# NVIDIAGameWorks/RayTracingDenoiser

Measured on AMD Instinct MI355X. Metric: Mpixels/s REBLUR_DIFFUSE_SPECULAR @1440p, higher is better.
Workload: dtype f32; 1 GPU; REBLUR_DIFFUSE_SPECULAR 2560x1440, default settings, analytic scene + 1rpp noise, moving camera; parallelism=1 GPU, storage=reference pool formats (fp16 history, R10G10B10A2 normals)

## Files before the change

raytracingdenoiser_amd/csrc/hip/kernels_reblur_history.hip:

```cpp
#include "passes.h"
#include "reblur_device.h"

namespace nrdhip {

constexpr int TILE_X = 32;
constexpr int TILE_Y = 8;

static const char* CheckSupportedHistory(const ReblurCB& c) {
    if (c.gRectOrigin.x != 0 || c.gRectOrigin.y != 0)
        return "internal error: a pass was handed a non-zero rectOrigin";
    if (c.gOrthoMode != 0.0f)
        return "REBLUR: orthographic projection is not supported (SURVEY.md section 8c)";
    return nullptr;
}

static_assert(TILE_X == 32 && TILE_Y == 8, "planes.h LoadBlockTileBytes: a workgroup covers two 16x16 tiles of one tile row");

namespace hf {
constexpr int BORDER = 2;
constexpr int BUF_X = TILE_X + 2 * BORDER;
constexpr int BUF_Y = TILE_Y + 2 * BORDER;
constexpr int BUF_STRIDE = BUF_X + 1;
}

struct HfPlanes {
    Plane tiles, normalRoughness, data1, viewZ, inDiff, inSpec, inDiffFast, inSpecFast, outDiff, outSpec, outDiffFast, outSpecFast;
    Plane inDiffSh, inSpecSh, outDiffSh, outSpecSh;
    NormalRoughnessGuide decodedNR;
};

struct HfPixel {
    int px, py, tx, ty;
    float viewZ, roughness, materialID, frustumSize;
    float3 N, Nv, Xv;
    float2 pixelUv;
};

template <bool IS_SPEC, bool DIFF, bool SPEC, bool PERF, int KIND, bool SH>
NRD_D typename ReblurSignal<KIND>::type HistoryFixSignal(const ReblurCB& c, const HfPlanes& P, const HfPixel& s, typename ReblurSignal<KIND>::type sig, float frameNum, float strideBase,
    const Plane& gIn_Signal, const Plane& gIn_Fast, const Plane& gOut_Fast, const float* s_Luma, float4& sh, const Plane& gIn_Sh) {
    typedef ReblurSignal<KIND> Sig;
    typedef typename Sig::type S;
    const int rw = c.gRectSizeMinusOne.x, rh = c.gRectSizeMinusOne.y;
    const float smc = GetSpecMagicCurve(s.roughness);

    float stride = strideBase * (frameNum < c.gHistoryFixFrameNum ? 1.0f : 0.0f);
    if (IS_SPEC)
        stride *= Lerp(0.5f, 1.0f, smc);
    stride = floorf(stride);

    if (stride != 0.0f) {
        const int stridei = (int)(stride + 0.5f);
        const float nonLinearAccumSpeed = Rcp(1.0f + frameNum);
        const float r = IS_SPEC ? s.roughness : 1.0f;
        const float2 rectSizeInv = ToF2(c.gRectSizeInv);
        const float4 hitDistParams = ToF4(c.gHitDistParams);

        float normalWeightParam = GetNormalWeightParam(nonLinearAccumSpeed, c.gLobeAngleFraction, r);
        float2 geometryWeightParams = GetGeometryWeightParams(c.gPlaneDistSensitivity, s.frustumSize, s.Xv, s.Nv);
        float2 relaxedRoughnessWeightParams = GetRelaxedRoughnessWeightParams(s.roughness * s.roughness, Sqrt(c.gRoughnessFraction));

        float hitDistScale = GetHitDistanceNormalization(s.viewZ, hitDistParams, r);
        float hitDist = ExtractHitDist(sig) * hitDistScale;
        float hitDistFactor = GetHitDistFactor(hitDist, s.frustumSize);
        float2 hitDistanceWeightParams = GetHitDistanceWeightParams(hitDistFactor, nonLinearAccumSpeed, r);

        float sumw = 1.0f + frameNum;
        if (PERF)
            sumw = 1.0f + Rcp(1.0f + c.gMaxAccumulatedFrameNum) - nonLinearAccumSpeed;
        sig = sig * sumw;
        if (SH)
            sh = F4(sh.x * sumw, sh.y * sumw, sh.z * sumw, IS_SPEC ? sh.w : sh.w * sumw);

        for (int j = -2; j <= 2; j++) {
            for (int i = -2; i <= 2; i++) {
                if ((i == 0 && j == 0) || (abs(i) + abs(j) == 4))
                    continue;

                float2 uv = s.pixelUv + F2(float(i), float(j)) * stride * rectSizeInv;
                int sx = ClampI(s.px + i * stridei, 0, rw), sy = ClampI(s.py + j * stridei, 0, rh);

                float zs = UnpackViewZ(c, LoadR32F(P.viewZ, sx, sy));
                float materialIDs;
                float4 Ns = LoadDecodedNormalRoughness(P.decodedNR, sx, sy, materialIDs);

                float angle = AcosApprox(Dot(Xyz(Ns), s.N));
                float3 Xvs = ReconstructViewPosition(uv, ToF4(c.gFrustum), zs, NRD_ORTHO_MODE(c));

                float w = IsInScreenNearest(uv);
                w *= ComputeWeight(Dot(s.Nv, Xvs), geometryWeightParams.x, geometryWeightParams.y);
                w *= CompareMaterials(s.materialID, materialIDs, IS_SPEC ? c.gSpecMinMaterial : c.gDiffMinMaterial) ? 1.0f : 0.0f;
                w *= ComputeExponentialWeight(angle, normalWeightParam, 0.0f);
                if (IS_SPEC)
                    w *= ComputeExponentialWeight(Ns.w * Ns.w, relaxedRoughnessWeightParams.x, relaxedRoughnessWeightParams.y);

                if (!PERF) {
                    float2 d1 = LoadData1<DIFF, SPEC>(P.data1, sx, sy);
                    w *= 1.0f + (IS_SPEC ? d1.y : d1.x);
                }

                S smp = Sig::Load(gIn_Signal, sx, sy);
                smp = Select(w == 0.0f, Sig::Zero(), smp);

                float hs = ExtractHitDist(smp) * hitDistScale;
                float hsFactor = GetHitDistFactor(hs, s.frustumSize);
                w *= ComputeExponentialWeight(hsFactor, hitDistanceWeightParams.x, hitDistanceWeightParams.y);

                if (IS_SPEC) {
                    float d = Div(Abs(hitDist - hs), Max(hitDist, hs) + 0.001f);
                    float b = LinearStep(0.03f, 0.05f, s.roughness);
                    w *= SmoothStep(0.2f + b, 0.05f + b, d);
                }

                sumw += w;
                sig = Mad(smp, w, sig);
                if (SH) {
                    float4 t = LoadRGBA16F(gIn_Sh, sx, sy);
                    t = Select(w == 0.0f, F4(0.0f), t);
                    sh = F4(sh.x + t.x * w, sh.y + t.y * w, sh.z + t.z * w, IS_SPEC ? sh.w : sh.w + t.w * w);
                }
            }
        }

        sumw = PositiveRcp(sumw);
        sig = sig * sumw;
        if (SH)
            sh = F4(sh.x * sumw, sh.y * sumw, sh.z * sumw, IS_SPEC ? sh.w : sh.w * sumw);
    }

    float center = s_Luma[(s.ty + hf::BORDER) * hf::BUF_STRIDE + s.tx + hf::BORDER];
    float m1 = center, m2 = center * center;

    float f = Sat(Div(frameNum, c.gHistoryFixFrameNum + NRD_EPS));
    if (IS_SPEC)
        f = Lerp(1.0f, f, smc);
    center = Lerp(GetLuma(sig), center, f);
    Sig::StoreFast(gOut_Fast, s.px, s.py, center);

#pragma unroll
    for (int j = 0; j <= 4; j++) {
#pragma unroll
        for (int i = 0; i <= 4; i++) {
            if (i == 2 && j == 2)
                continue;
            float d = s_Luma[(s.ty + j) * hf::BUF_STRIDE + s.tx + i];
            m1 += d;
            m2 += d * d;
        }
    }

    float luma = GetLuma(sig);

    if (KIND == SIGNAL_RADIANCE && c.gAntiFirefly != 0.0f) {
        float am1 = 0.0f, am2 = 0.0f;
        const int R = PERF ? 3 : REBLUR_ANTI_FIREFLY_FILTER_RADIUS;
        for (int j = -R; j <= R; j++)
            for (int i = -R; i <= R; i++) {
                if (abs(i) <= 1 && abs(j) <= 1)
                    continue;
                float d = LoadR16F(gIn_Fast, ClampI(s.px + i, 0, rw), ClampI(s.py + j, 0, rh));
                am1 += d;
                am2 += d * d;
            }
        float invNorm = Rcp(float((R * 2 + 1) * (R * 2 + 1) - 3 * 3));
        am1 *= invNorm;
        am2 *= invNorm;
        float sigma = Sqrt(Abs(am2 - am1 * am1)) * REBLUR_ANTI_FIREFLY_SIGMA_SCALE;
        luma = Clamp(luma, am1 - sigma, am1 + sigma);
    }

    m1 = m1 * (1.0f / 25.0f);
    m2 = m2 * (1.0f / 25.0f);
    float sigma = Sqrt(Abs(m2 - m1 * m1)) * (KIND != SIGNAL_RADIANCE ? REBLUR_COLOR_CLAMPING_SIGMA_SCALE_OCCLUSION : REBLUR_COLOR_CLAMPING_SIGMA_SCALE);
    float lumaClamped = Clamp(luma, m1 - sigma, m1 + sigma);
    luma = Lerp(lumaClamped, luma, Rcp(1.0f + (c.gMaxFastAccumulatedFrameNum < c.gMaxAccumulatedFrameNum ? 1.0f : 0.0f) * frameNum * 2.0f));

    if (SH) {
        float k = GetLumaScale(Length(Xyz(sh)), luma);
        sh = F4(sh.x * k, sh.y * k, sh.z * k, sh.w);
    }
    return ChangeLuma(sig, luma);
}

#ifndef NRD_REBLUR_HF_ROTATE
#define NRD_REBLUR_HF_ROTATE 1
#endif
template <bool DIFF, bool SPEC, bool PERF, int KIND, bool SH>
__global__ __launch_bounds__(TILE_X* TILE_Y, SH ? 0 : NRD_WAVES_REBLUR_HF) void ReblurHistoryFixKernel(ReblurCB c, HfPlanes P, RowRange rr) {
    typedef ReblurSignal<KIND> Sig;
    typedef typename Sig::type S;
    __shared__ float s_DiffLuma[DIFF ? hf::BUF_Y * hf::BUF_STRIDE : 1];
    __shared__ float s_SpecLuma[SPEC ? hf::BUF_Y * hf::BUF_STRIDE : 1];

    const int tx = threadIdx.x % TILE_X, ty = threadIdx.x / TILE_X;
    const int blockY = BlockTileY(rr);
    const int tileX = NRD_REBLUR_HF_ROTATE ? BlockTileXRotated(rr, blockY) : BlockTileX(rr);
    const int px = tileX * TILE_X + tx, py = blockY * TILE_Y + ty;
    const int rw = c.gRectSizeMinusOne.x, rh = c.gRectSizeMinusOne.y;

    const uint32_t tileBytes = LoadBlockTileBytes(P.tiles, tileX, blockY);
    if (!TileBytesHaveGeometry<2>(tileBytes))
        return;
    const int qx = min(px, rw), qy = min(max(py, 0), rh);
    const bool preSky = TileByteIsSky(tileBytes, tx >> 4);
    const float preViewZ = LoadR32F(P.viewZ, qx, qy);
    float preMaterialID;
    const float4 preNormalAndRoughness = LoadDecodedNormalRoughness(P.decodedNR, qx, qy, preMaterialID);
    const float2 preData1 = LoadData1<DIFF, SPEC>(P.data1, qx, qy);
    S preDiff = Sig::Zero(), preSpec = Sig::Zero();
    if (DIFF)
        preDiff = Sig::Load(P.inDiff, qx, qy);
    if (SPEC)
        preSpec = Sig::Load(P.inSpec, qx, qy);
    {
        const int baseX = tileX * TILE_X - hf::BORDER, baseY = blockY * TILE_Y - hf::BORDER;
        for (int i = threadIdx.x; i < hf::BUF_X * hf::BUF_Y; i += TILE_X * TILE_Y) {
            int lx = i % hf::BUF_X, ly = i / hf::BUF_X;
            int gx = ClampI(baseX + lx, 0, rw), gy = ClampI(baseY + ly, 0, rh);
            if (DIFF)
                s_DiffLuma[ly * hf::BUF_STRIDE + lx] = Sig::LoadFast(P.inDiffFast, gx, gy);
            if (SPEC)
                s_SpecLuma[ly * hf::BUF_STRIDE + lx] = Sig::LoadFast(P.inSpecFast, gx, gy);
        }
    }
    __syncthreads();

    if (px > rw || py > rh || py < rr.rowBegin || py >= rr.rowEnd)
        return;
    if (preSky)
        return;
    HfPixel s;
    s.viewZ = UnpackViewZ(c, preViewZ);
    if (s.viewZ > c.gDenoisingRange)
        return;

    s.px = px, s.py = py, s.tx = tx, s.ty = ty;
    s.materialID = preMaterialID;
    float4 normalAndRoughness = preNormalAndRoughness;
    s.N = Xyz(normalAndRoughness);
    s.roughness = normalAndRoughness.w;
    s.frustumSize = GetFrustumSize(c.gMinRectDimMulUnproject, NRD_ORTHO_MODE(c), s.viewZ);
    s.pixelUv = F2(float(px) + 0.5f, float(py) + 0.5f) * ToF2(c.gRectSizeInv);
    s.Xv = ReconstructViewPosition(s.pixelUv, ToF4(c.gFrustum), s.viewZ, NRD_ORTHO_MODE(c));
    s.Nv = RotateVectorInverse(c.gViewToWorld, s.N);
    float2 frameNum = preData1;
    float2 stride = F2(Div(c.gHistoryFixBasePixelStride, 2.0f + frameNum.x), Div(c.gHistoryFixBasePixelStride, 2.0f + frameNum.y));

    if (DIFF) {
        float4 diffSh = F4(0.0f);
        if (SH)
            diffSh = LoadRGBA16F(P.inDiffSh, px, py);
        S diff = HistoryFixSignal<false, DIFF, SPEC, PERF, KIND, SH>(c, P, s, preDiff, frameNum.x, stride.x, P.inDiff, P.inDiffFast, P.outDiffFast, s_DiffLuma, diffSh, P.inDiffSh);
        Sig::Store(P.outDiff, px, py, diff);
        if (SH)
            StoreRGBA16F(P.outDiffSh, px, py, diffSh);
    }
    if (SPEC) {
        float4 specSh = F4(0.0f);
        if (SH)
            specSh = LoadRGBA16F(P.inSpecSh, px, py);
        S spec = HistoryFixSignal<true, DIFF, SPEC, PERF, KIND, SH>(c, P, s, preSpec, frameNum.y, stride.y, P.inSpec, P.inSpecFast, P.outSpecFast, s_SpecLuma, specSh, P.inSpecSh);
        Sig::Store(P.outSpec, px, py, spec);
        if (SH)
            StoreRGBA16F(P.outSpecSh, px, py, specSh);
    }
}

template <bool DIFF, bool SPEC, bool PERF, int KIND, bool SH>
static const char* LaunchHistoryFix(const PassArgs& a) {
    const ReblurCB& c = *(const ReblurCB*)a.constants;
    if (const char* err = CheckSupportedHistory(c))
        return err;
    HfPlanes P = {};
    uint32_t k = 0;
    P.tiles = a.planes[k++];
    P.normalRoughness = a.planes[k++];
    if (const char* err = MakeNormalRoughnessGuide(a, P.decodedNR))
        return err;
    P.data1 = a.planes[k++];
    P.viewZ = a.planes[k++];
    if (DIFF) P.inDiff = a.planes[k++];
    if (SPEC) P.inSpec = a.planes[k++];
    if (DIFF) P.inDiffFast = a.planes[k++];
    if (SPEC) P.inSpecFast = a.planes[k++];
    if (DIFF && SH) P.inDiffSh = a.planes[k++];
    if (SPEC && SH) P.inSpecSh = a.planes[k++];
    if (DIFF) P.outDiff = a.planes[k++];
    if (SPEC) P.outSpec = a.planes[k++];
    if (DIFF) P.outDiffFast = a.planes[k++];
    if (SPEC) P.outSpecFast = a.planes[k++];
    if (DIFF && SH) P.outDiffSh = a.planes[k++];
    if (SPEC && SH) P.outSpecSh = a.planes[k++];
    if (k != a.planesNum)
        return "REBLUR history fix: unexpected resource count";
    RowGrid g = GridForRows(c.gRectSizeMinusOne.x + 1, c.gRectSizeMinusOne.y + 1, TILE_X, TILE_Y, a.rowBegin, a.rowEnd);
    LaunchPass(a, (ReblurHistoryFixKernel<DIFF, SPEC, PERF, KIND, SH>), g.grid, dim3(TILE_X * TILE_Y), c, P, MakeRowRange(g));
    return nullptr;
}

namespace ts {
constexpr int BORDER = 1;
constexpr int BUF_X = TILE_X + 2 * BORDER;
constexpr int BUF_Y = TILE_Y + 2 * BORDER;
constexpr int BUF_STRIDE = BUF_X + 1;
}

struct TsPlanes {
    Plane tiles, normalRoughness, viewZ, data1, data2, inDiff, inSpec, historyDiffLuma, historySpecLuma, inSpecHitDistForTracking, mv, outInternalData, outDiff, outSpec, outDiffLuma,
        outSpecLuma;
    Plane inDiffSh, inSpecSh, outDiffSh, outSpecSh;
    NormalRoughnessGuide decodedNR;
    Plane baseColorMetalness;
};

template <bool PERF>
NRD_D void LumaStats(const ReblurCB& c, const float* s_Luma, int tx, int ty, float& luma, float& m1, float& sigma) {
    luma = s_Luma[(ty + ts::BORDER) * ts::BUF_STRIDE + tx + ts::BORDER];
    float M1 = luma, M2 = luma * luma, mn = NRD_INF, mx = -NRD_INF;
#pragma unroll
    for (int j = 0; j <= 2; j++) {
#pragma unroll
        for (int i = 0; i <= 2; i++) {
            if (i == 1 && j == 1)
                continue;
            float d = s_Luma[(ty + j) * ts::BUF_STRIDE + tx + i];
            M1 += d;
            M2 += d * d;
            mn = Min(mn, d);
            mx = Max(mx, d);
        }
    }
    M1 = M1 * (1.0f / 9.0f);
    M2 = M2 * (1.0f / 9.0f);
    m1 = M1;
    sigma = Sqrt(Abs(M2 - M1 * M1));
    if (!PERF && c.gMaxBlurRadius != 0.0f)
        luma = Clamp(luma, mn, mx);
}

template <bool DIFF, bool SPEC, bool PERF, bool SH, int KIND, bool MVMOD>
__global__ __launch_bounds__(TILE_X* TILE_Y, NRD_WAVES_REBLUR_TS) void ReblurTemporalStabilizationKernel(ReblurCB c, TsPlanes P, RowRange rr) {
    typedef ReblurSignal<KIND> Sig;
    typedef typename Sig::type S;
    __shared__ float s_DiffLuma[DIFF ? ts::BUF_Y * ts::BUF_STRIDE : 1];
    __shared__ float s_SpecLuma[SPEC ? ts::BUF_Y * ts::BUF_STRIDE : 1];

    const int tx = threadIdx.x % TILE_X, ty = threadIdx.x / TILE_X;
    const int blockY = BlockTileY(rr, NRD_ALT_TILE_ORDER != 0);
    const int px = BlockTileX(rr) * TILE_X + tx, py = blockY * TILE_Y + ty;
// ... 281 lines not shown
```

raytracingdenoiser_amd/csrc/hip/kernels_relax_spatial.hip:

```cpp
#include "relax_device.h"

namespace nrdhip {

namespace {

constexpr int TILE_X = RELAX_TILE_X;
constexpr int TILE_Y = RELAX_TILE_Y;

__device__ __constant__ const float g_Poisson8[8][3] = {
    {-0.4706069f, -0.4427112f, +0.6461146f}, {-0.9057375f, +0.3003471f, +0.9542373f}, {-0.3487388f, +0.4037880f, +0.5335386f}, {+0.1023042f, +0.6439373f, +0.6520134f},
    {+0.5699277f, +0.3513750f, +0.6695386f}, {+0.2939128f, -0.1131226f, +0.3149309f}, {+0.7836658f, -0.4208784f, +0.8895339f}, {+0.1564120f, -0.8198990f, +0.8346850f}};

__device__ __constant__ const float g_Poisson8Gaussian[8] = {0.7591725f, 0.5482766f, 0.8287159f, 0.7553454f, 0.743887f, 0.9366367f, 0.59319115f, 0.6313964f};

__global__ __launch_bounds__(256) void RelaxClassifyTilesKernel(Plane viewZ, Plane tiles, float denoisingRange, int tilesPerRow, int tileRows) {
    const int wave = threadIdx.x >> 6, lane = threadIdx.x & 63;
    const int tileIndex = blockIdx.x * 4 + wave;
    if (tileIndex >= tilesPerRow * tileRows)
        return;
    const int tx = tileIndex % tilesPerRow, ty = tileIndex / tilesPerRow;
    const int x = tx * 16 + (lane & 3) * 4, y = ty * 16 + (lane >> 2);

    bool allSky = true;
    if (y < viewZ.h && x + 3 < viewZ.w) {
// ... 397 lines not shown
            StoreRGBA16FHinted<NT>(P.spec.outSh, px, py, Clamp4(specularSH, -NRD_FP16_MAX, NRD_FP16_MAX));
    }
}

template <bool DIFF, bool SPEC, bool SH>
const char* LaunchPrePass(const PassArgs& a) {
    if (const char* e = CheckSupportedRelax(a))
        return e;
    PlaneCursor cur(a);
    PrePassPlanes P = {};
    P.tiles = cur.next();
    if (SPEC) P.spec.in = cur.next();
    if (DIFF) P.diff.in = cur.next();
    P.normalRoughness = cur.next();
    P.viewZ = cur.next();
    if (SH && SPEC) P.spec.inSh = cur.next();
    if (SH && DIFF) P.diff.inSh = cur.next();
    if (SPEC) P.spec.out = cur.next();
    if (DIFF) P.diff.out = cur.next();
    if (SH && SPEC) P.spec.outSh = cur.next();
    if (SH && DIFF) P.diff.outSh = cur.next();
    P.decodedNR = a.decodedNormalRoughness;
    P.worldPos = a.worldPosViewZ;
    if (!cur.complete() || !P.decodedNR.ptr)
        return "RELAX PrePass: unexpected resource count or missing decoded normal/roughness cache";
    RelaxCB c = LoadRelaxConstants(a);
    RowGrid g = GridForRows(c.shared.gRectSize.x, c.shared.gRectSize.y, TILE_X, TILE_Y, a.rowBegin, a.rowEnd);
    const char* forceGeneric = getenv("NRD_HIP_GENERIC_TAPS");
    const bool fullRect = c.shared.gResolutionScale.x == 1.0f && c.shared.gResolutionScale.y == 1.0f && c.shared.gRectSize.x == P.decodedNR.w &&
                          c.shared.gRectSize.y == P.decodedNR.h && P.viewZ.w == P.decodedNR.w && P.viewZ.h == P.decodedNR.h && !(forceGeneric && atoi(forceGeneric) != 0);
    if ((SPEC && c.shared.gSpecCheckerboard != 2u) || (DIFF && c.shared.gDiffCheckerboard != 2u))
        LaunchPass(a, (RelaxPrePassKernel<DIFF, SPEC, SH, true, false>), g.grid, dim3(256), P, c, MakeRowRange(g));
    else if (fullRect && !(c.shared.gSpecMinMaterial < 3.0f || c.shared.gDiffMinMaterial < 3.0f) && (uint32_t)P.decodedNR.w * (uint32_t)P.decodedNR.h > NRD_NT_STORE_PIXELS)
        LaunchPass(a, (RelaxPrePassKernel<DIFF, SPEC, SH, false, true, false, true>), g.grid, dim3(256), P, c, MakeRowRange(g));
    else if (fullRect && !(c.shared.gSpecMinMaterial < 3.0f || c.shared.gDiffMinMaterial < 3.0f))
        LaunchPass(a, (RelaxPrePassKernel<DIFF, SPEC, SH, false, true, false>), g.grid, dim3(256), P, c, MakeRowRange(g));
    else if (fullRect)
        LaunchPass(a, (RelaxPrePassKernel<DIFF, SPEC, SH, false, true>), g.grid, dim3(256), P, c, MakeRowRange(g));
    else
        LaunchPass(a, (RelaxPrePassKernel<DIFF, SPEC, SH, false, false>), g.grid, dim3(256), P, c, MakeRowRange(g));
    return nullptr;
}

struct HistoryFixPlanes {
    Plane tiles, historyLength, normalRoughness, viewZ;
    Plane decodedNR;
    SignalPlanes spec, diff;
};

#ifndef NRD_RELAX_HF_ROTATE
#define NRD_RELAX_HF_ROTATE 1
#endif
template <bool DIFF, bool SPEC, bool SH>
__global__ __launch_bounds__(256, NRD_WAVES_RELAX_HF) void RelaxHistoryFixKernel(HistoryFixPlanes P, RelaxCB c, RowRange rows) {
    const int blockY = BlockTileY(rows, false) ;
    const int tileX = NRD_RELAX_HF_ROTATE ? BlockTileXRotated(rows, blockY) : BlockTileX(rows);
    const uint32_t tileBytes = LoadBlockTileBytes(P.tiles, tileX, blockY);
    if (!TileBytesHaveGeometry<2>(tileBytes))
        return;
    const int px = tileX * TILE_X + (threadIdx.x & 31), py = blockY * TILE_Y + (threadIdx.x >> 5);
    const int rectW = c.shared.gRectSize.x, rectH = c.shared.gRectSize.y;
    if (px >= rectW || py >= rectH || py < rows.rowBegin || py >= rows.rowEnd)
        return;
    float centerViewZ = RelaxUnpackViewZ(c, LoadR32F(P.viewZ, px, py));
    float historyLength = 255.0f * LoadR8Unorm(P.historyLength, px, py);
    if (TileByteIsSky(tileBytes, (threadIdx.x & 31) >> 4))
        return;
    if (centerViewZ > c.shared.gDenoisingRange || (historyLength > c.shared.gHistoryFixFrameNum || c.shared.gHistoryFixFrameNum == 1.0f))
        return;

    float centerMaterialID;
    float4 centerNormalRoughness = LoadDecodedNormalRoughness(P.decodedNR, px, py, centerMaterialID);
    float3 centerNormal = Xyz(centerNormalRoughness);
    float centerRoughness = centerNormalRoughness.w;
    float3 centerWorldPos = GetCurrentWorldPosFromPixelPos(c, px, py, centerViewZ);
    float3 centerV = -Normalize(centerWorldPos);
    float depthThreshold = c.shared.gDepthThreshold * centerViewZ;

    float4 diffuseSum = DIFF ? LoadRGBA16F(P.diff.in, px, py) : F4(0.0f);
    float4 diffuseSumSH = (DIFF && SH) ? LoadRGBA16F(P.diff.inSh, px, py) : F4(0.0f);
    float diffuseWSum = 1.0f;
    float4 specularSum = SPEC ? LoadRGBA16F(P.spec.in, px, py) : F4(0.0f);
    float4 specularSumSH = (SPEC && SH) ? LoadRGBA16F(P.spec.inSh, px, py) : F4(0.0f);
    float roughnessModified = specularSumSH.w;
    float specularWSum = 1.0f;
    float2 specularNormalWeightParams = SPEC ? GetNormalWeightParams_ATrous(centerRoughness, 5.0f, 1.0f, 0.0f, c.shared.gLobeAngleFraction, c.shared.gSpecLobeAngleSlack) : F2(0.0f, 0.0f);
    const float normalPower = Max(c.shared.gHistoryFixEdgeStoppingNormalPower, 0.01f);

    float r = Div(c.shared.gHistoryFixBasePixelStride, 1.0f + historyLength);
    r = floorf(r + 0.5f);

    for (int j = -2; j <= 2; j++)
        for (int i = -2; i <= 2; i++) {
            int dx = (int)(float(i) * r), dy = (int)(float(j) * r);
            int sx = px + dx, sy = py + dy;
            bool isInside = sx >= 0 && sy >= 0 && sx < rectW && sy < rectH;
            if (i == 0 && j == 0)
                continue;

            float sampleMaterialID;
            float3 sampleNormal = Xyz(LoadDecodedNormalRoughnessOrZero(P.decodedNR, sx, sy, sampleMaterialID));
            float sampleViewZ = RelaxUnpackViewZ(c, LoadR32FOrZero(P.viewZ, sx, sy));
            float3 sampleWorldPos = GetCurrentWorldPosFromPixelPos(c, sx, sy, sampleViewZ);
            float geometryWeight = GetPlaneDistanceWeight_Atrous(centerWorldPos, centerNormal, sampleWorldPos, depthThreshold);

            if (DIFF) {
                float diffuseW = geometryWeight;
                diffuseW *= Pow(Max(0.01f, Dot(centerNormal, sampleNormal)), normalPower);
                diffuseW = isInside ? diffuseW : 0.0f;
                diffuseW *= Cmp(CompareMaterials(sampleMaterialID, centerMaterialID, c.shared.gDiffMinMaterial));
                if (diffuseW > 1e-4f) {
                    diffuseSum = diffuseSum + LoadRGBA16FOrZero(P.diff.in, sx, sy) * diffuseW;
                    if (SH)
                        diffuseSumSH = diffuseSumSH + LoadRGBA16FOrZero(P.diff.inSh, sx, sy) * diffuseW;
                    diffuseWSum += diffuseW;
                }
            }
            if (SPEC) {
                float3 sampleV = -Normalize(sampleWorldPos + c.shared.gRoughnessEdgeStoppingRelaxation * centerWorldPos);
                float specularW = geometryWeight;
                specularW *= GetSpecularNormalWeight_ATrous(specularNormalWeightParams, centerNormal, sampleNormal, centerV, sampleV);
                specularW = isInside ? specularW : 0.0f;
                specularW *= Cmp(CompareMaterials(sampleMaterialID, centerMaterialID, c.shared.gSpecMinMaterial));
                if (specularW > 1e-4f) {
                    specularSum = specularSum + LoadRGBA16FOrZero(P.spec.in, sx, sy) * specularW;
                    if (SH)
                        specularSumSH = specularSumSH + LoadRGBA16FOrZero(P.spec.inSh, sx, sy) * specularW;
                    specularWSum += specularW;
                }
            }
        }

    if (DIFF) {
        StoreRGBA16F(P.diff.out, px, py, Div(diffuseSum, diffuseWSum));
        if (SH)
            StoreRGBA16F(P.diff.outSh, px, py, Div(diffuseSumSH, diffuseWSum));
    }
    if (SPEC) {
        StoreRGBA16F(P.spec.out, px, py, Div(specularSum, specularWSum));
        if (SH)
            StoreRGBA16F(P.spec.outSh, px, py, F4(Div(Xyz(specularSumSH), specularWSum), roughnessModified));
    }
}

template <bool DIFF, bool SPEC, bool SH>
const char* LaunchHistoryFix(const PassArgs& a) {
    if (const char* e = CheckSupportedRelax(a))
        return e;
    PlaneCursor cur(a);
    HistoryFixPlanes P = {};
    P.tiles = cur.next();
    if (SPEC) P.spec.in = cur.next();
    if (DIFF) P.diff.in = cur.next();
    P.historyLength = cur.next();
    P.normalRoughness = cur.next();
    P.viewZ = cur.next();
    if (SH && SPEC) P.spec.inSh = cur.next();
    if (SH && DIFF) P.diff.inSh = cur.next();
    if (SPEC) P.spec.out = cur.next();
    if (DIFF) P.diff.out = cur.next();
    if (SH && SPEC) P.spec.outSh = cur.next();
    if (SH && DIFF) P.diff.outSh = cur.next();
    P.decodedNR = a.decodedNormalRoughness;
    if (!cur.complete() || !P.decodedNR.ptr)
        return "RELAX HistoryFix: unexpected resource count or missing decoded normal/roughness cache";
    RelaxCB c = LoadRelaxConstants(a);
    RowGrid g = GridForRows(c.shared.gRectSize.x, c.shared.gRectSize.y, TILE_X, TILE_Y, a.rowBegin, a.rowEnd);
    LaunchPass(a, (RelaxHistoryFixKernel<DIFF, SPEC, SH>), g.grid, dim3(256), P, c, MakeRowRange(g));
    return nullptr;
}

struct CopyPlanes {
    SignalPlanes spec, diff;
};

template <bool DIFF, bool SPEC>
__global__ __launch_bounds__(256) void RelaxCopyKernel(CopyPlanes P, int gridW, int gridH) {
    const int px = blockIdx.x * TILE_X + (threadIdx.x & 31), py = blockIdx.y * TILE_Y + (threadIdx.x >> 5);
    if (px >= gridW || py >= gridH)
        return;
    if (SPEC && InBounds(P.spec.out, px, py))
        StoreRGBA16F(P.spec.out, px, py, LoadRGBA16FOrZero(P.spec.in, px, py));
    if (DIFF && InBounds(P.diff.out, px, py))
        StoreRGBA16F(P.diff.out, px, py, LoadRGBA16FOrZero(P.diff.in, px, py));
}

template <bool DIFF, bool SPEC>
const char* LaunchCopy(const PassArgs& a) {
    if (const char* e = CheckSupportedRelax(a))
        return e;
    PlaneCursor cur(a);
    CopyPlanes P = {};
    if (SPEC) P.spec.in = cur.next();
    if (DIFF) P.diff.in = cur.next();
    if (SPEC) P.spec.out = cur.next();
    if (DIFF) P.diff.out = cur.next();
    if (!cur.complete())
        return "RELAX Copy: unexpected resource count";
    RelaxCB c = LoadRelaxConstants(a);
    const int gridW = (c.shared.gRectSize.x + 7) & ~7, gridH = (c.shared.gRectSize.y + 7) & ~7;
    LaunchPass(a, (RelaxCopyKernel<DIFF, SPEC>), GridFor(gridW, gridH, TILE_X, TILE_Y), dim3(256), P, gridW, gridH);
    return nullptr;
}

struct AntiFireflyPlanes {
    Plane tiles, viewZ, decodedNR;
    SignalPlanes spec, diff;
};

template <bool IS_SPEC>
NRD_D void AntiFireflySignal(const RelaxCB& c, const SignalPlanes& S, const Plane& decodedNR, int px, int py, float centerMaterialID) {
    const int rectW = c.shared.gRectSize.x, rectH = c.shared.gRectSize.y;
    const float minMaterial = IS_SPEC ? c.shared.gSpecMinMaterial : c.shared.gDiffMinMaterial;
    const float4 center = LoadRGBA16F(S.in, px, py);
    const float centerLuminance = Luminance(Xyz(center));
    float maxLuminance = -1.0f, minLuminance = 1.0e6f;
    float3 maxValue = Xyz(center), minValue = Xyz(center);
#pragma unroll
    for (int yy = -1; yy <= 1; yy++)
#pragma unroll
        for (int xx = -1; xx <= 1; xx++) {
// ... 160 lines not shown
```

raytracingdenoiser_amd/csrc/hip/passes.h:

```cpp
#pragma once

#include "planes.h"

#include <hip/hip_runtime.h>

#include <cstdlib>
#include <cstring>
#include <utility>
#include <vector>

#ifndef NRD_WAVES_REBLUR_SPATIAL
#define NRD_WAVES_REBLUR_SPATIAL 0
#endif
#ifndef NRD_WAVES_REBLUR_HF
#define NRD_WAVES_REBLUR_HF 5
#endif
#ifndef NRD_WAVES_REBLUR_TS
#define NRD_WAVES_REBLUR_TS 0
#endif
#ifndef NRD_WAVES_RELAX_ATROUS
#define NRD_WAVES_RELAX_ATROUS 0
#endif
#ifndef NRD_WAVES_RELAX_ATROUS_SMEM
#define NRD_WAVES_RELAX_ATROUS_SMEM 0
#endif
#ifndef NRD_WAVES_RELAX_PREPASS
#define NRD_WAVES_RELAX_PREPASS 0
#endif
#ifndef NRD_WAVES_RELAX_TA
#define NRD_WAVES_RELAX_TA 3
#endif
#ifndef NRD_WAVES_RELAX_HC
#define NRD_WAVES_RELAX_HC 0
#endif
#ifndef NRD_WAVES_RELAX_HF
#define NRD_WAVES_RELAX_HF 0
#endif
#ifndef NRD_RELAX_PREPASS_UNROLL
#define NRD_RELAX_PREPASS_UNROLL 2
#endif

namespace nrdhip {

struct MotionParams {
    float worldToClipPrev[16];
    float viewToWorld[16];
    float frustum[4];
    float frustumRight[4], frustumUp[4], frustumForward[4];
    float mvScale[4];
    float rectSizeInv[2];
    float rectHeightPrev, viewZScale, denoisingRange;
    int rectW, rectH, relaxForm;
};
void LaunchMotionRows(hipStream_t stream, const Plane& viewZ, const Plane& mv, const MotionParams& p, int rowBegin, int rowEnd, uint32_t* outMaxBits);

struct LaunchRecord {
    const void* func;
    dim3 grid, block;
    std::vector<uint8_t> args;
    std::vector<uint32_t> offsets;
    void (*launch)(const LaunchRecord&, hipStream_t);
};
struct LaunchRecorder {
    bool keep = false;
    uint32_t count = 0;
    std::vector<LaunchRecord> records;
};

// ... 111 lines not shown
            }
    }
    if (g.bandTiles && stripe > 1) {
        g.stripeTiles = stripe < g.bandTiles ? stripe : g.bandTiles;
        g.bandTiles = ((g.bandTiles + g.stripeTiles - 1) / g.stripeTiles) * g.stripeTiles;
    }
    g.grid = dim3((unsigned)(g.bandTiles ? 8 * g.bandTiles : tilesX), (unsigned)(ny > 0 ? ny : 1), 1);
    return g;
}
struct RowRange {
    int firstBlockY, rowBegin, rowEnd;
    int bandTiles;
    int stripeTiles;
};
inline RowRange MakeRowRange(const RowGrid& g) { return RowRange{g.firstBlockY, g.rowBegin, g.rowEnd, g.bandTiles, g.stripeTiles}; }
#ifndef NRD_ALT_TILE_ORDER
#define NRD_ALT_TILE_ORDER 0
#endif
#ifndef NRD_REVERSE_TILE_ROWS
#define NRD_REVERSE_TILE_ROWS -1
#endif
__device__ __forceinline__ int BlockTileY(const RowRange& r, bool bottomUp = false) {
    const bool reverse = NRD_REVERSE_TILE_ROWS < 0 ? bottomUp : NRD_REVERSE_TILE_ROWS != 0;
    return r.firstBlockY + (reverse ? (int)(gridDim.y - 1u - blockIdx.y) : (int)blockIdx.y);
}
#ifndef NRD_XCD_STAIRCASE_ROWS
#define NRD_XCD_STAIRCASE_ROWS 0
#endif
__device__ __forceinline__ int BlockTileXPlain(const RowRange& r) {
    const unsigned bx = blockIdx.x;
    if (!r.bandTiles)
        return (int)bx;
    const unsigned xcd = bx & 7u, j = bx >> 3;
    if (r.stripeTiles == r.bandTiles)
        return (int)(xcd * (unsigned)r.bandTiles + j);
    const unsigned stripe = j / (unsigned)r.stripeTiles, within = j - stripe * (unsigned)r.stripeTiles;
    return (int)((stripe * 8u + xcd) * (unsigned)r.stripeTiles + within);
}
__device__ __forceinline__ int BlockTileX(const RowRange& r) {
    const int t = BlockTileXPlain(r);
    if (NRD_XCD_STAIRCASE_ROWS == 0 || !r.bandTiles)
        return t;
    const unsigned blockY = (unsigned)BlockTileY(r);
    return (int)(((unsigned)t + (blockY / (unsigned)(NRD_XCD_STAIRCASE_ROWS ? NRD_XCD_STAIRCASE_ROWS : 1)) * (unsigned)r.stripeTiles) % gridDim.x);
}

__device__ __forceinline__ int BlockTileXRotated(const RowRange& r, int blockY) {
    const int t = BlockTileXPlain(r);
    if (!r.bandTiles)
        return t;
    return (int)(((unsigned)t + (unsigned)blockY * (unsigned)r.stripeTiles) % gridDim.x);
}

}
```

Before: 5293 Mpixels/s.

## Add compacted job queue for history-fix pixels to reduce wave divergence

Adds an optional intra-block job queue to the REBLUR and RELAX history-fix kernels. Pixels that need reconstruction are compacted with wave ballots and redistributed across lanes, and the results are passed back through shared memory, so sparse young-history pixels no longer leave waves mostly idle. The queue is gated by an env var that defaults to 0, so by default the new path is skipped. It also raises the REBLUR HF occupancy hint from 5 to 6 waves, which applies by default. In exchange, the kernel now reserves extra shared memory for the queue and carries more register state, which could cost occupancy.

Measured after the change: 5293 Mpixels/s (median of 2 runs). About the same (+0.0%).

```diff
diff --git a/raytracingdenoiser_amd/csrc/hip/kernels_reblur_history.hip b/raytracingdenoiser_amd/csrc/hip/kernels_reblur_history.hip
--- a/raytracingdenoiser_amd/csrc/hip/kernels_reblur_history.hip
+++ b/raytracingdenoiser_amd/csrc/hip/kernels_reblur_history.hip
@@ -36,97 +36,140 @@
     float2 pixelUv;
 };
 
+template <bool IS_SPEC>
+NRD_D float HistoryFixStride(const ReblurCB& c, float roughness, float frameNum, float strideBase) {
+    float stride = strideBase * (frameNum < c.gHistoryFixFrameNum ? 1.0f : 0.0f);
+    if (IS_SPEC)
+        stride *= Lerp(0.5f, 1.0f, GetSpecMagicCurve(roughness));
+    return floorf(stride);
+}
+
+NRD_D HfPixel MakeHfPixel(const ReblurCB& c, int px, int py, int tx, int ty, float viewZ, float4 normalAndRoughness, float materialID) {
+    HfPixel s;
+    s.viewZ = viewZ;
+    s.px = px, s.py = py, s.tx = tx, s.ty = ty;
+    s.materialID = materialID;
+    s.N = Xyz(normalAndRoughness);
+    s.roughness = normalAndRoughness.w;
+    s.frustumSize = GetFrustumSize(c.gMinRectDimMulUnproject, NRD_ORTHO_MODE(c), s.viewZ);
+    s.pixelUv = F2(float(px) + 0.5f, float(py) + 0.5f) * ToF2(c.gRectSizeInv);
+    s.Xv = ReconstructViewPosition(s.pixelUv, ToF4(c.gFrustum), s.viewZ, NRD_ORTHO_MODE(c));
+    s.Nv = RotateVectorInverse(c.gViewToWorld, s.N);
+    return s;
+}
+
 template <bool IS_SPEC, bool DIFF, bool SPEC, bool PERF, int KIND, bool SH>
-NRD_D typename ReblurSignal<KIND>::type HistoryFixSignal(const ReblurCB& c, const HfPlanes& P, const HfPixel& s, typename ReblurSignal<KIND>::type sig, float frameNum, float strideBase,
-    const Plane& gIn_Signal, const Plane& gIn_Fast, const Plane& gOut_Fast, const float* s_Luma, float4& sh, const Plane& gIn_Sh) {
+NRD_D void HistoryFixReconstruct(const ReblurCB& c, const HfPlanes& P, const HfPixel& s, typename ReblurSignal<KIND>::type& sig, float frameNum, float stride, const Plane& gIn_Signal,
+    float4& sh, const Plane& gIn_Sh) {
+    typedef ReblurSignal<KIND> Sig;
+    typedef typename Sig::type S;
+    const int rw = c.gRectSizeMinusOne.x, rh = c.gRectSizeMinusOne.y;
+    const int stridei = (int)(stride + 0.5f);
+    const float nonLinearAccumSpeed = Rcp(1.0f + frameNum);
+    const float r = IS_SPEC ? s.roughness : 1.0f;
+    const float2 rectSizeInv = ToF2(c.gRectSizeInv);
+    const float4 hitDistParams = ToF4(c.gHitDistParams);
+
+    float normalWeightParam = GetNormalWeightParam(nonLinearAccumSpeed, c.gLobeAngleFraction, r);
+    float2 geometryWeightParams = GetGeometryWeightParams(c.gPlaneDistSensitivity, s.frustumSize, s.Xv, s.Nv);
+    float2 relaxedRoughnessWeightParams = GetRelaxedRoughnessWeightParams(s.roughness * s.roughness, Sqrt(c.gRoughnessFraction));
+
+    float hitDistScale = GetHitDistanceNormalization(s.viewZ, hitDistParams, r);
+    float hitDist = ExtractHitDist(sig) * hitDistScale;
+    float hitDistFactor = GetHitDistFactor(hitDist, s.frustumSize);
+    float2 hitDistanceWeightParams = GetHitDistanceWeightParams(hitDistFactor, nonLinearAccumSpeed, r);
+
+    float sumw = 1.0f + frameNum;
+    if (PERF)
+        sumw = 1.0f + Rcp(1.0f + c.gMaxAccumulatedFrameNum) - nonLinearAccumSpeed;
+    sig = sig * sumw;
+    if (SH)
+        sh = F4(sh.x * sumw, sh.y * sumw, sh.z * sumw, IS_SPEC ? sh.w : sh.w * sumw);
+
+    for (int j = -2; j <= 2; j++) {
+        for (int i = -2; i <= 2; i++) {
+            if ((i == 0 && j == 0) || (abs(i) + abs(j) == 4))
+                continue;
+
+            float2 uv = s.pixelUv + F2(float(i), float(j)) * stride * rectSizeInv;
+            int sx = ClampI(s.px + i * stridei, 0, rw), sy = ClampI(s.py + j * stridei, 0, rh);
+
+            float zs = UnpackViewZ(c, LoadR32F(P.viewZ, sx, sy));
+            float materialIDs;
+            float4 Ns = LoadDecodedNormalRoughness(P.decodedNR, sx, sy, materialIDs);
+
+            float angle = AcosApprox(Dot(Xyz(Ns), s.N));
+            float3 Xvs = ReconstructViewPosition(uv, ToF4(c.gFrustum), zs, NRD_ORTHO_MODE(c));
+
+            float w = IsInScreenNearest(uv);
+            w *= ComputeWeight(Dot(s.Nv, Xvs), geometryWeightParams.x, geometryWeightParams.y);
+            w *= CompareMaterials(s.materialID, materialIDs, IS_SPEC ? c.gSpecMinMaterial : c.gDiffMinMaterial) ? 1.0f : 0.0f;
+            w *= ComputeExponentialWeight(angle, normalWeightParam, 0.0f);
+            if (IS_SPEC)
+                w *= ComputeExponentialWeight(Ns.w * Ns.w, relaxedRoughnessWeightParams.x, relaxedRoughnessWeightParams.y);
+
+            if (!PERF) {
+                float2 d1 = LoadData1<DIFF, SPEC>(P.data1, sx, sy);
+                w *= 1.0f + (IS_SPEC ? d1.y : d1.x);
+            }
+
+            S smp = Sig::Load(gIn_Signal, sx, sy);
+            smp = Select(w == 0.0f, Sig::Zero(), smp);
+
+            float hs = ExtractHitDist(smp) * hitDistScale;
+            float hsFactor = GetHitDistFactor(hs, s.frustumSize);
+            w *= ComputeExponentialWeight(hsFactor, hitDistanceWeightParams.x, hitDistanceWeightParams.y);
+
+            if (IS_SPEC) {
+                float d = Div(Abs(hitDist - hs), Max(hitDist, hs) + 0.001f);
+                float b = LinearStep(0.03f, 0.05f, s.roughness);
+                w *= SmoothStep(0.2f + b, 0.05f + b, d);
+            }
+
+            sumw += w;
+            sig = Mad(smp, w, sig);
+            if (SH) {
+                float4 t = LoadRGBA16F(gIn_Sh, sx, sy);
+                t = Select(w == 0.0f, F4(0.0f), t);
+                sh = F4(sh.x + t.x * w, sh.y + t.y * w, sh.z + t.z * w, IS_SPEC ? sh.w : sh.w + t.w * w);
+            }
+        }
+    }
+
+    sumw = PositiveRcp(sumw);
+    sig = sig * sumw;
+    if (SH)
+        sh = F4(sh.x * sumw, sh.y * sumw, sh.z * sumw, IS_SPEC ? sh.w : sh.w * sumw);
+}
+
+template <bool IS_SPEC, bool DIFF, bool SPEC, bool PERF, int KIND, bool SH>
+NRD_D void HistoryFixJob(const ReblurCB& c, const HfPlanes& P, int tileX, int blockY, uint32_t owner, const Plane& gIn_Signal, const Plane& gIn_Sh, typename ReblurSignal<KIND>::type& outSignal,
+    float4& outSh) {
+    typedef ReblurSignal<KIND> Sig;
+    const int px = tileX * TILE_X + int(owner % TILE_X), py = blockY * TILE_Y + int(owner / TILE_X);
+    float materialID;
+    const float4 normalAndRoughness = LoadDecodedNormalRoughness(P.decodedNR, px, py, materialID);
+    const HfPixel s = MakeHfPixel(c, px, py, 0, 0, UnpackViewZ(c, LoadR32F(P.viewZ, px, py)), normalAndRoughness, materialID);
+    const float2 data1 = LoadData1<DIFF, SPEC>(P.data1, px, py);
+    const float frameNum = IS_SPEC ? data1.y : data1.x;
+    const float stride = HistoryFixStride<IS_SPEC>(c, s.roughness, frameNum, Div(c.gHistoryFixBasePixelStride, 2.0f + frameNum));
+    typename Sig::type sig = Sig::Load(gIn_Signal, px, py);
+    float4 sh = F4(0.0f);
+    if (SH)
+        sh = LoadRGBA16F(gIn_Sh, px, py);
+    HistoryFixReconstruct<IS_SPEC, DIFF, SPEC, PERF, KIND, SH>(c, P, s, sig, frameNum, stride, gIn_Signal, sh, gIn_Sh);
+    outSignal = sig;
+    if (SH)
+        outSh = sh;
+}
+
+template <bool IS_SPEC, bool DIFF, bool SPEC, bool PERF, int KIND, bool SH>
+NRD_D typename ReblurSignal<KIND>::type HistoryFixSignal(const ReblurCB& c, const HfPlanes& P, const HfPixel& s, typename ReblurSignal<KIND>::type sig, float frameNum, const Plane& gIn_Fast,
+    const Plane& gOut_Fast, const float* s_Luma, float4& sh) {
     typedef ReblurSignal<KIND> Sig;
     typedef typename Sig::type S;
     const int rw = c.gRectSizeMinusOne.x, rh = c.gRectSizeMinusOne.y;
     const float smc = GetSpecMagicCurve(s.roughness);
-
-    float stride = strideBase * (frameNum < c.gHistoryFixFrameNum ? 1.0f : 0.0f);
-    if (IS_SPEC)
-        stride *= Lerp(0.5f, 1.0f, smc);
-    stride = floorf(stride);
-
-    if (stride != 0.0f) {
-        const int stridei = (int)(stride + 0.5f);
-        const float nonLinearAccumSpeed = Rcp(1.0f + frameNum);
-        const float r = IS_SPEC ? s.roughness : 1.0f;
-        const float2 rectSizeInv = ToF2(c.gRectSizeInv);
-        const float4 hitDistParams = ToF4(c.gHitDistParams);
-
-        float normalWeightParam = GetNormalWeightParam(nonLinearAccumSpeed, c.gLobeAngleFraction, r);
-        float2 geometryWeightParams = GetGeometryWeightParams(c.gPlaneDistSensitivity, s.frustumSize, s.Xv, s.Nv);
-        float2 relaxedRoughnessWeightParams = GetRelaxedRoughnessWeightParams(s.roughness * s.roughness, Sqrt(c.gRoughnessFraction));
-
-        float hitDistScale = GetHitDistanceNormalization(s.viewZ, hitDistParams, r);
-        float hitDist = ExtractHitDist(sig) * hitDistScale;
-        float hitDistFactor = GetHitDistFactor(hitDist, s.frustumSize);
-        float2 hitDistanceWeightParams = GetHitDistanceWeightParams(hitDistFactor, nonLinearAccumSpeed, r);
-
-        float sumw = 1.0f + frameNum;
-        if (PERF)
-            sumw = 1.0f + Rcp(1.0f + c.gMaxAccumulatedFrameNum) - nonLinearAccumSpeed;
-        sig = sig * sumw;
-        if (SH)
-            sh = F4(sh.x * sumw, sh.y * sumw, sh.z * sumw, IS_SPEC ? sh.w : sh.w * sumw);
-
-        for (int j = -2; j <= 2; j++) {
-            for (int i = -2; i <= 2; i++) {
-                if ((i == 0 && j == 0) || (abs(i) + abs(j) == 4))
-                    continue;
-
-                float2 uv = s.pixelUv + F2(float(i), float(j)) * stride * rectSizeInv;
-                int sx = ClampI(s.px + i * stridei, 0, rw), sy = ClampI(s.py + j * stridei, 0, rh);
-
-                float zs = UnpackViewZ(c, LoadR32F(P.viewZ, sx, sy));
-                float materialIDs;
-                float4 Ns = LoadDecodedNormalRoughness(P.decodedNR, sx, sy, materialIDs);
-
-                float angle = AcosApprox(Dot(Xyz(Ns), s.N));
-                float3 Xvs = ReconstructViewPosition(uv, ToF4(c.gFrustum), zs, NRD_ORTHO_MODE(c));
-
-                float w = IsInScreenNearest(uv);
-                w *= ComputeWeight(Dot(s.Nv, Xvs), geometryWeightParams.x, geometryWeightParams.y);
-                w *= CompareMaterials(s.materialID, materialIDs, IS_SPEC ? c.gSpecMinMaterial : c.gDiffMinMaterial) ? 1.0f : 0.0f;
-                w *= ComputeExponentialWeight(angle, normalWeightParam, 0.0f);
-                if (IS_SPEC)
-                    w *= ComputeExponentialWeight(Ns.w * Ns.w, relaxedRoughnessWeightParams.x, relaxedRoughnessWeightParams.y);
-
-                if (!PERF) {
-                    float2 d1 = LoadData1<DIFF, SPEC>(P.data1, sx, sy);
-                    w *= 1.0f + (IS_SPEC ? d1.y : d1.x);
-                }
-
-                S smp = Sig::Load(gIn_Signal, sx, sy);
-                smp = Select(w == 0.0f, Sig::Zero(), smp);
-
-                float hs = ExtractHitDist(smp) * hitDistScale;
-                float hsFactor = GetHitDistFactor(hs, s.frustumSize);
-                w *= ComputeExponentialWeight(hsFactor, hitDistanceWeightParams.x, hitDistanceWeightParams.y);
-
-                if (IS_SPEC) {
-                    float d = Div(Abs(hitDist - hs), Max(hitDist, hs) + 0.001f);
-                    float b = LinearStep(0.03f, 0.05f, s.roughness);
-                    w *= SmoothStep(0.2f + b, 0.05f + b, d);
-                }
-
-                sumw += w;
-                sig = Mad(smp, w, sig);
-                if (SH) {
-                    float4 t = LoadRGBA16F(gIn_Sh, sx, sy);
-                    t = Select(w == 0.0f, F4(0.0f), t);
-                    sh = F4(sh.x + t.x * w, sh.y + t.y * w, sh.z + t.z * w, IS_SPEC ? sh.w : sh.w + t.w * w);
-                }
-            }
-        }
-
-        sumw = PositiveRcp(sumw);
-        sig = sig * sumw;
-        if (SH)
-            sh = F4(sh.x * sumw, sh.y * sumw, sh.z * sumw, IS_SPEC ? sh.w : sh.w * sumw);
-    }
 
     float center = s_Luma[(s.ty + hf::BORDER) * hf::BUF_STRIDE + s.tx + hf::BORDER];
     float m1 = center, m2 = center * center;
@@ -186,11 +229,18 @@
 #define NRD_REBLUR_HF_ROTATE 1
 #endif
 template <bool DIFF, bool SPEC, bool PERF, int KIND, bool SH>
-__global__ __launch_bounds__(TILE_X* TILE_Y, SH ? 0 : NRD_WAVES_REBLUR_HF) void ReblurHistoryFixKernel(ReblurCB c, HfPlanes P, RowRange rr) {
+__global__ __launch_bounds__(TILE_X* TILE_Y, SH ? 0 : NRD_WAVES_REBLUR_HF) void ReblurHistoryFixKernel(ReblurCB c, HfPlanes P, RowRange rr, int queueCapacity) {
     typedef ReblurSignal<KIND> Sig;
     typedef typename Sig::type S;
     __shared__ float s_DiffLuma[DIFF ? hf::BUF_Y * hf::BUF_STRIDE : 1];
     __shared__ float s_SpecLuma[SPEC ? hf::BUF_Y * hf::BUF_STRIDE : 1];
+    constexpr int QUEUES = (DIFF ? 1 : 0) + (SPEC ? 1 : 0), SPEC_Q = QUEUES - 1;
+    constexpr uint32_t DIFF_WAVES = SPEC ? 2u : 4u, SPEC_WAVES = DIFF ? 2u : 4u;
+    static_assert(HF_QUEUE_MAX == TILE_X * TILE_Y, "one job per lane");
+    __shared__ uint32_t s_JobCount[4];
+    __shared__ uint8_t s_JobOwner[QUEUES][TILE_X * TILE_Y];
+    __shared__ S s_JobSignal[QUEUES][HF_QUEUE_MAX / QUEUES];
+    __shared__ float4 s_JobSh[SH ? QUEUES : 1][SH ? HF_QUEUE_MAX / QUEUES : 1];
 
     const int tx = threadIdx.x % TILE_X, ty = threadIdx.x / TILE_X;
     const int blockY = BlockTileY(rr);
@@ -223,34 +273,73 @@
                 s_SpecLuma[ly * hf::BUF_STRIDE + lx] = Sig::LoadFast(P.inSpecFast, gx, gy);
         }
     }
+    const float viewZ = UnpackViewZ(c, preViewZ);
+    const bool valid = !(px > rw || py > rh || py < rr.rowBegin || py >= rr.rowEnd) && !preSky && !(viewZ > c.gDenoisingRange);
+    const float2 frameNum = preData1;
+    const float2 strideBase = F2(Div(c.gHistoryFixBasePixelStride, 2.0f + frameNum.x), Div(c.gHistoryFixBasePixelStride, 2.0f + frameNum.y));
+    const float diffStride = DIFF ? HistoryFixStride<false>(c, preNormalAndRoughness.w, frameNum.x, strideBase.x) : 0.0f;
+    const float specStride = SPEC ? HistoryFixStride<true>(c, preNormalAndRoughness.w, frameNum.y, strideBase.y) : 0.0f;
+    const uint32_t wave = threadIdx.x >> 6;
+    uint32_t diffRank = 0u, specRank = 0u;
+    if (queueCapacity > 0) {
+        uint32_t n = 0u;
+        if (DIFF)
+            n = PushWaveJobs(valid && diffStride != 0.0f, s_JobOwner[0], diffRank);
+        if (SPEC)
+            n |= PushWaveJobs(valid && specStride != 0.0f, s_JobOwner[SPEC_Q], specRank) << 16;
+        if ((threadIdx.x & 63u) == 0u)
+            s_JobCount[wave] = n;
+    }
     __syncthreads();
 
-    if (px > rw || py > rh || py < rr.rowBegin || py >= rr.rowEnd)
+    bool queued = false;
+    uint32_t diffJob = 0u, specJob = 0u;
+    if (queueCapacity > 0) {
+        uint32_t diffCount[4], specCount[4], diffTotal = 0u, specTotal = 0u;
+        for (uint32_t w = 0; w < 4u; w++) {
+            const uint32_t n = s_JobCount[w];
+            diffCount[w] = n & 0xFFFFu, specCount[w] = n >> 16;
+            diffJob += w < wave ? diffCount[w] : 0u, specJob += w < wave ? specCount[w] : 0u;
+            diffTotal += diffCount[w], specTotal += specCount[w];
+        }
+        diffJob += diffRank, specJob += specRank;
+        diffTotal = NRD_WAVE_UNIFORM(diffTotal), specTotal = NRD_WAVE_UNIFORM(specTotal);
+        queued = diffTotal + specTotal != 0u && diffTotal + specTotal <= (uint32_t)queueCapacity && diffTotal <= 64u * DIFF_WAVES && specTotal <= 64u * SPEC_WAVES;
+        if (queued) {
+            const uint32_t lane = threadIdx.x & 63u;
+            if (DIFF && wave < DIFF_WAVES) {
+                const uint32_t job = lane * DIFF_WAVES + wave;
+                if (job < diffTotal)
+                    HistoryFixJob<false, DIFF, SPEC, PERF, KIND, SH>(c, P, tileX, blockY, JobOwner(s_JobOwner[0], diffCount, job), P.inDiff, P.inDiffSh, s_JobSignal[0][job], s_JobSh[0][SH ? job : 0]);
+            }
+            if (SPEC && wave >= 4u - SPEC_WAVES) {
+                const uint32_t job = lane * SPEC_WAVES + (wave - (4u - SPEC_WAVES));
+                if (job < specTotal)
+                    HistoryFixJob<true, DIFF, SPEC, PERF, KIND, SH>(c, P, tileX, blockY, JobOwner(s_JobOwner[SPEC_Q], specCount, job), P.inSpec, P.inSpecSh, s_JobSignal[SPEC_Q][job],
+                        s_JobSh[SH ? SPEC_Q : 0][SH ? job : 0]);
+            }
+            __syncthreads();
+        }
+    }
+
+    if (!valid)
         return;
-    if (preSky)
-        return;
-    HfPixel s;
-    s.viewZ = UnpackViewZ(c, preViewZ);
-    if (s.viewZ > c.gDenoisingRange)
-        return;
-
-    s.px = px, s.py = py, s.tx = tx, s.ty = ty;
-    s.materialID = preMaterialID;
-    float4 normalAndRoughness = preNormalAndRoughness;
-    s.N = Xyz(normalAndRoughness);
-    s.roughness = normalAndRoughness.w;
-    s.frustumSize = GetFrustumSize(c.gMinRectDimMulUnproject, NRD_ORTHO_MODE(c), s.viewZ);
-    s.pixelUv = F2(float(px) + 0.5f, float(py) + 0.5f) * ToF2(c.gRectSizeInv);
-    s.Xv = ReconstructViewPosition(s.pixelUv, ToF4(c.gFrustum), s.viewZ, NRD_ORTHO_MODE(c));
-    s.Nv = RotateVectorInverse(c.gViewToWorld, s.N);
-    float2 frameNum = preData1;
-    float2 stride = F2(Div(c.gHistoryFixBasePixelStride, 2.0f + frameNum.x), Div(c.gHistoryFixBasePixelStride, 2.0f + frameNum.y));
+    const HfPixel s = MakeHfPixel(c, px, py, tx, ty, viewZ, preNormalAndRoughness, preMaterialID);
 
     if (DIFF) {
         float4 diffSh = F4(0.0f);
         if (SH)
             diffSh = LoadRGBA16F(P.inDiffSh, px, py);
-        S diff = HistoryFixSignal<false, DIFF, SPEC, PERF, KIND, SH>(c, P, s, preDiff, frameNum.x, stride.x, P.inDiff, P.inDiffFast, P.outDiffFast, s_DiffLuma, diffSh, P.inDiffSh);
+        S diff = preDiff;
+        if (diffStride != 0.0f) {
+            if (queued) {
+                diff = s_JobSignal[0][diffJob];
+                if (SH)
+                    diffSh = s_JobSh[0][diffJob];
+            } else
+                HistoryFixReconstruct<false, DIFF, SPEC, PERF, KIND, SH>(c, P, s, diff, frameNum.x, diffStride, P.inDiff, diffSh, P.inDiffSh);
+        }
+        diff = HistoryFixSignal<false, DIFF, SPEC, PERF, KIND, SH>(c, P, s, diff, frameNum.x, P.inDiffFast, P.outDiffFast, s_DiffLuma, diffSh);
         Sig::Store(P.outDiff, px, py, diff);
         if (SH)
             StoreRGBA16F(P.outDiffSh, px, py, diffSh);
@@ -259,7 +348,16 @@
         float4 specSh = F4(0.0f);
         if (SH)
             specSh = LoadRGBA16F(P.inSpecSh, px, py);
-        S spec = HistoryFixSignal<true, DIFF, SPEC, PERF, KIND, SH>(c, P, s, preSpec, frameNum.y, stride.y, P.inSpec, P.inSpecFast, P.outSpecFast, s_SpecLuma, specSh, P.inSpecSh);
+        S spec = preSpec;
+        if (specStride != 0.0f) {
+            if (queued) {
+                spec = s_JobSignal[SPEC_Q][specJob];
+                if (SH)
+                    specSh = s_JobSh[SPEC_Q][specJob];
+            } else
+                HistoryFixReconstruct<true, DIFF, SPEC, PERF, KIND, SH>(c, P, s, spec, frameNum.y, specStride, P.inSpec, specSh, P.inSpecSh);
+        }
+        spec = HistoryFixSignal<true, DIFF, SPEC, PERF, KIND, SH>(c, P, s, spec, frameNum.y, P.inSpecFast, P.outSpecFast, s_SpecLuma, specSh);
         Sig::Store(P.outSpec, px, py, spec);
         if (SH)
             StoreRGBA16F(P.outSpecSh, px, py, specSh);
@@ -294,7 +392,7 @@
     if (k != a.planesNum)
         return "REBLUR history fix: unexpected resource count";
     RowGrid g = GridForRows(c.gRectSizeMinusOne.x + 1, c.gRectSizeMinusOne.y + 1, TILE_X, TILE_Y, a.rowBegin, a.rowEnd);
-    LaunchPass(a, (ReblurHistoryFixKernel<DIFF, SPEC, PERF, KIND, SH>), g.grid, dim3(TILE_X * TILE_Y), c, P, MakeRowRange(g));
+    LaunchPass(a, (ReblurHistoryFixKernel<DIFF, SPEC, PERF, KIND, SH>), g.grid, dim3(TILE_X * TILE_Y), c, P, MakeRowRange(g), HistoryFixQueueCapacity());
     return nullptr;
 }
 
diff --git a/raytracingdenoiser_amd/csrc/hip/kernels_relax_spatial.hip b/raytracingdenoiser_amd/csrc/hip/kernels_relax_spatial.hip
--- a/raytracingdenoiser_amd/csrc/hip/kernels_relax_spatial.hip
+++ b/raytracingdenoiser_amd/csrc/hip/kernels_relax_spatial.hip
@@ -473,23 +473,8 @@
 #define NRD_RELAX_HF_ROTATE 1
 #endif
 template <bool DIFF, bool SPEC, bool SH>
-__global__ __launch_bounds__(256, NRD_WAVES_RELAX_HF) void RelaxHistoryFixKernel(HistoryFixPlanes P, RelaxCB c, RowRange rows) {
-    const int blockY = BlockTileY(rows, false) ;
-    const int tileX = NRD_RELAX_HF_ROTATE ? BlockTileXRotated(rows, blockY) : BlockTileX(rows);
-    const uint32_t tileBytes = LoadBlockTileBytes(P.tiles, tileX, blockY);
-    if (!TileBytesHaveGeometry<2>(tileBytes))
-        return;
-    const int px = tileX * TILE_X + (threadIdx.x & 31), py = blockY * TILE_Y + (threadIdx.x >> 5);
+NRD_D void RelaxHistoryFixPixel(const HistoryFixPlanes& P, const RelaxCB& c, int px, int py, float centerViewZ, float historyLength) {
     const int rectW = c.shared.gRectSize.x, rectH = c.shared.gRectSize.y;
-    if (px >= rectW || py >= rectH || py < rows.rowBegin || py >= rows.rowEnd)
-        return;
-    float centerViewZ = RelaxUnpackViewZ(c, LoadR32F(P.viewZ, px, py));
-    float historyLength = 255.0f * LoadR8Unorm(P.historyLength, px, py);
-    if (TileByteIsSky(tileBytes, (threadIdx.x & 31) >> 4))
-        return;
-    if (centerViewZ > c.shared.gDenoisingRange || (historyLength > c.shared.gHistoryFixFrameNum || c.shared.gHistoryFixFrameNum == 1.0f))
-        return;
-
     float centerMaterialID;
     float4 centerNormalRoughness = LoadDecodedNormalRoughness(P.decodedNR, px, py, centerMaterialID);
     float3 centerNormal = Xyz(centerNormalRoughness);
@@ -564,6 +549,52 @@
     }
 }
 
+NRD_D bool RelaxHistoryFixIsYoung(const HistoryFixPlanes& P, const RelaxCB& c, int px, int py, float& centerViewZ, float& historyLength) {
+    centerViewZ = RelaxUnpackViewZ(c, LoadR32F(P.viewZ, px, py));
+    historyLength = 255.0f * LoadR8Unorm(P.historyLength, px, py);
+    return !(centerViewZ > c.shared.gDenoisingRange || (historyLength > c.shared.gHistoryFixFrameNum || c.shared.gHistoryFixFrameNum == 1.0f));
+}
+
+template <bool DIFF, bool SPEC, bool SH>
+__global__ __launch_bounds__(256, NRD_WAVES_RELAX_HF) void RelaxHistoryFixKernel(HistoryFixPlanes P, RelaxCB c, RowRange rows, int queueCapacity) {
+    __shared__ uint32_t s_JobCount[4];
+    __shared__ uint8_t s_JobOwner[256];
+
+    const int blockY = BlockTileY(rows, false) ;
+    const int tileX = NRD_RELAX_HF_ROTATE ? BlockTileXRotated(rows, blockY) : BlockTileX(rows);
+    const uint32_t tileBytes = LoadBlockTileBytes(P.tiles, tileX, blockY);
+    if (!TileBytesHaveGeometry<2>(tileBytes))
+        return;
+    const int px = tileX * TILE_X + (threadIdx.x & 31), py = blockY * TILE_Y + (threadIdx.x >> 5);
+    const int rectW = c.shared.gRectSize.x, rectH = c.shared.gRectSize.y;
+    float centerViewZ, historyLength;
+    bool young = RelaxHistoryFixIsYoung(P, c, min(px, rectW - 1), min(py, rectH - 1), centerViewZ, historyLength);
+    young = young && !(px >= rectW || py >= rectH || py < rows.rowBegin || py >= rows.rowEnd) && !TileByteIsSky(tileBytes, (threadIdx.x & 31) >> 4);
+
+    if (queueCapacity > 0) {
+        const uint32_t wave = threadIdx.x >> 6;
+        uint32_t rank;
+        const uint32_t n = PushWaveJobs(young, s_JobOwner, rank);
+        if ((threadIdx.x & 63u) == 0u)
+            s_JobCount[wave] = n;
+        __syncthreads();
+        const uint32_t counts[4] = {s_JobCount[0], s_JobCount[1], s_JobCount[2], s_JobCount[3]};
+        const uint32_t total = NRD_WAVE_UNIFORM(counts[0] + counts[1] + counts[2] + counts[3]);
+        if (total <= (uint32_t)queueCapacity) {
+            const uint32_t job = (threadIdx.x & 63u) * 4u + wave;
+            if (job >= total)
+                return;
+            const uint32_t owner = JobOwner(s_JobOwner, counts, job);
+            const int ox = tileX * TILE_X + int(owner & 31u), oy = blockY * TILE_Y + int(owner >> 5);
+            RelaxHistoryFixIsYoung(P, c, ox, oy, centerViewZ, historyLength);
+            RelaxHistoryFixPixel<DIFF, SPEC, SH>(P, c, ox, oy, centerViewZ, historyLength);
+            return;
+        }
+    }
+    if (young)
+        RelaxHistoryFixPixel<DIFF, SPEC, SH>(P, c, px, py, centerViewZ, historyLength);
+}
+
 template <bool DIFF, bool SPEC, bool SH>
 const char* LaunchHistoryFix(const PassArgs& a) {
     if (const char* e = CheckSupportedRelax(a))
@@ -587,7 +618,7 @@
         return "RELAX HistoryFix: unexpected resource count or missing decoded normal/roughness cache";
     RelaxCB c = LoadRelaxConstants(a);
     RowGrid g = GridForRows(c.shared.gRectSize.x, c.shared.gRectSize.y, TILE_X, TILE_Y, a.rowBegin, a.rowEnd);
-    LaunchPass(a, (RelaxHistoryFixKernel<DIFF, SPEC, SH>), g.grid, dim3(256), P, c, MakeRowRange(g));
+    LaunchPass(a, (RelaxHistoryFixKernel<DIFF, SPEC, SH>), g.grid, dim3(256), P, c, MakeRowRange(g), HistoryFixQueueCapacity());
     return nullptr;
 }
 
diff --git a/raytracingdenoiser_amd/csrc/hip/passes.h b/raytracingdenoiser_amd/csrc/hip/passes.h
--- a/raytracingdenoiser_amd/csrc/hip/passes.h
+++ b/raytracingdenoiser_amd/csrc/hip/passes.h
@@ -13,7 +13,7 @@
 #define NRD_WAVES_REBLUR_SPATIAL 0
 #endif
 #ifndef NRD_WAVES_REBLUR_HF
-#define NRD_WAVES_REBLUR_HF 5
+#define NRD_WAVES_REBLUR_HF 6
 #endif
 #ifndef NRD_WAVES_REBLUR_TS
 #define NRD_WAVES_REBLUR_TS 0
@@ -231,4 +231,48 @@
     return (int)(((unsigned)t + (unsigned)blockY * (unsigned)r.stripeTiles) % gridDim.x);
 }
 
-}
+constexpr int HF_QUEUE_MAX = 256;
+#ifndef NRD_HF_QUEUE_DEFAULT
+#define NRD_HF_QUEUE_DEFAULT 0
+#endif
+inline int HistoryFixQueueCapacity() {
+    const char* e = getenv("NRD_HIP_HF_QUEUE");
+    const int v = e ? atoi(e) : NRD_HF_QUEUE_DEFAULT;
+    return v < 0 ? 0 : (v > HF_QUEUE_MAX ? HF_QUEUE_MAX : v);
+}
+#ifndef NRD_WAVE_UNIFORM
+#define NRD_WAVE_UNIFORM(x) __builtin_amdgcn_readfirstlane(x)
+#endif
+struct WaveRank {
+    uint32_t rank, count;
+};
+__device__ __forceinline__ WaveRank RankInWave(bool flag) {
+    const uint32_t lane = threadIdx.x & 63u, bit = 1u << (lane & 31u);
+    uint32_t mine = flag ? bit : 0u;
+    for (int m = 1; m < 32; m <<= 1)
+        mine |= __shfl_xor(mine, m);
+    const uint32_t other = __shfl_xor(mine, 32);
+    const uint32_t below = (uint32_t)__builtin_popcount(mine & (bit - 1u));
+    WaveRank r;
+    r.rank = lane < 32u ? below : below + (uint32_t)__builtin_popcount(other);
+    r.count = (uint32_t)__builtin_popcount(mine) + (uint32_t)__builtin_popcount(other);
+    return r;
+}
+__device__ __forceinline__ uint32_t PushWaveJobs(bool flag, uint8_t* owners, uint32_t& rank) {
+    rank = 0u;
+    if (!__any(flag))
+        return 0u;
+    const WaveRank r = RankInWave(flag);
+    rank = r.rank;
+    if (flag)
+        owners[(threadIdx.x & ~63u) + r.rank] = (uint8_t)threadIdx.x;
+    return r.count;
+}
+__device__ __forceinline__ uint32_t JobOwner(const uint8_t* owners, const uint32_t counts[4], uint32_t job) {
+    uint32_t w = 0u;
+    for (; w < 3u && job >= counts[w]; w++)
+        job -= counts[w];
+    return owners[w * 64u + job];
+}
+
+}
```
